# Low-power/THUNDER

Measured on AMD Instinct MI355X. Metric: particle-images/sec through expectation (box 256, 2000 rot samples), higher is better.
Workload: dtype f32 (global scan: FP32 operands split exactly into three bf16, six products -- dropped terms <= 2^-24 |w||T| each, comparable to an FP32 product's rounding -- FP32 accumulation, cancellation-guarded direct FP32 recompute; phases: FP32); 1 GPU; C3: 3D refine box 256, 2000 rotation x 151 translation global scan at rU=24 (nPxl=870) + 10 particle-filter phases (125 x 9); images_per_gpu=12500, global_batch=12500, box=256, pf=2, nR=2000, nT=151, nPxl=870, scan_algo=4, perturb_mean=acg, parallelism=dp1 (hemisphere = rank % 2)

## Files before the change

### thunder_amd/csrc/scan_split.hip

```cpp
#include "internal.h"
#include "scan_common.h"

namespace {

typedef float f32x16 __attribute__((ext_vector_type(16)));
typedef float f32x4v __attribute__((ext_vector_type(4)));
typedef __bf16 bf16x8 __attribute__((ext_vector_type(8)));
typedef __bf16 bf16x2 __attribute__((ext_vector_type(2)));
typedef uint32_t u32x4 __attribute__((ext_vector_type(4)));

enum Mode { BF16X3 = 0, BF16X6 = 2 };
typedef __bf16 H;
typedef bf16x8 HV;

template <int MODE> constexpr int nplane() { return MODE == BF16X6 ? 3 : 2; }

constexpr float SCAN_GUARD = 4.f;
constexpr int GCAP = 32;

constexpr int KC = 16;
static_assert(KC % 16 == 0, "whole float4 rows per thread in the stagers");
constexpr int IMG_TILE = 64;
constexpr int ROT_TILE = 8;
constexpr int THREADS = 64 * ROT_TILE;
constexpr int NWAVE = ROT_TILE;
constexpr int TROW = KC * 2 + 8;
constexpr int APITCH = KC + 2;

inline int pad_to(int v, int m) { return (v + m - 1) / m * m; }

struct Dims {
    int nImg, nR, nT, nPxl, nImgPad, nPxlPad, nTPad, nRB, nCk, nRBias;
};

Dims dims(int nImg, int nR, int nT, int nPxl)
{
    Dims d;
    d.nImg = nImg; d.nR = nR; d.nT = nT; d.nPxl = nPxl;
    d.nImgPad = pad_to(nImg, IMG_TILE);
    d.nPxlPad = pad_to(nPxl, KC);
    d.nTPad = pad_to(nT, 32);
    d.nRB = (nR + ROT_TILE - 1) / ROT_TILE;
    d.nCk = d.nPxlPad / KC;
    d.nRBias = pad_to(nR, 64);
    return d;
}

struct WS {
    float2* Ac;
    float* Bc;
    float* Aconst;
    float* bias;
    uint16_t* Thi;
    uint16_t* Tlo;
    uint16_t* Tl2;
    float2* Pc;
    float2* wRp;
    float* pM;
    float* pWT;
    float* pTf;
    size_t bytes;
};

WS carve(void* base, const Dims& d)
{
    thx::Carver c(base, ~size_t(0));
    WS w;
    w.Ac = c.take<float2>((size_t)d.nCk * d.nImgPad * APITCH);
    w.Bc = c.take<float>((size_t)d.nPxlPad * d.nImgPad);
    w.Aconst = c.take<float>(d.nImgPad);
    w.bias = c.take<float>((size_t)d.nImgPad * d.nRBias);
    w.Thi = c.take<uint16_t>((size_t)d.nCk * d.nTPad * TROW);
    w.Tlo = c.take<uint16_t>((size_t)d.nCk * d.nTPad * TROW);
    w.Tl2 = c.take<uint16_t>((size_t)d.nCk * d.nTPad * TROW);
    w.Pc = c.take<float2>((size_t)d.nCk * d.nRB * ROT_TILE * KC);
    w.wRp = c.take<float2>((size_t)d.nImg * d.nR);
    w.pM = c.take<float>((size_t)d.nRB * d.nImgPad);
    w.pWT = c.take<float>((size_t)d.nRB * d.nImgPad * d.nTPad);
    w.pTf = c.take<float>(d.nTPad);
    w.bytes = c.off + 256;
    return w;
}

template <typename H>
THX_DEV void split16(float x, H& hi, H& lo)
{
    hi = (H)x;
    lo = (H)(x - (float)hi);
}

THX_DEV void split3(float x, __bf16& hi, __bf16& mid, __bf16& lo)
{
    hi = (__bf16)x;
    const float r = x - (float)hi;
    mid = (__bf16)r;
    lo = (__bf16)(r - (float)mid);
}

typedef float f2v __attribute__((ext_vector_type(2)));
THX_DEV void split3x2(f2v x, uint32_t& hi, uint32_t& mid, uint32_t& lo)
{
    auto pk = [](float a, float b) { return __builtin_bit_cast(uint32_t, bf16x2{(__bf16)a, (__bf16)b}); };
    auto unpk = [](uint32_t v) { return f2v{__uint_as_float(v << 16), __uint_as_float(v & 0xffff0000u)}; };
    hi = pk(x.x, x.y);
    asm volatile("" : "+v"(hi));
    const f2v r = x - unpk(hi);
    mid = pk(r.x, r.y);
    asm volatile("" : "+v"(mid));
    const f2v r2 = r - unpk(mid);
    lo = pk(r2.x, r2.y);
}

__global__ void __launch_bounds__(256) k_prep_aconst(const float2* __restrict__ dat,
                                                     const float* __restrict__ sig, int nImg,
                                                     int nPxl, int nImgPad,
                                                     float* __restrict__ Aconst)
{
    const int l = blockIdx.x * 4 + (threadIdx.x >> 6);
    const int lane = threadIdx.x & 63;
    if (l >= nImgPad) return;
    float a = 0.f;
    if (l < nImg)
        for (int i = lane; i < nPxl; i += 64) {
            const size_t s = (size_t)l * nPxl + i;
            const float2 d = dat[s];
            a += sig[s] * (d.x * d.x + d.y * d.y);
        }
    a = wave_sum(a);
    if (lane == 0) Aconst[l] = a;
}

__global__ void __launch_bounds__(256) k_prep_img(const float2* __restrict__ dat,
                                                  const float* __restrict__ ctf,
                                                  const float* __restrict__ sig,
                                                  int nImg,
                                                  int nPxl, int nImgPad, int nPxlPad,
                                                  float2* __restrict__ Ac,
                                                  float* __restrict__ Bc)
{
    const long n = (long)nImgPad * nPxlPad;
    for (long q = blockIdx.x * (long)blockDim.x + threadIdx.x; q < n;
         q += (long)gridDim.x * blockDim.x) {
        const int i = (int)(q % nPxlPad), l = (int)(q / nPxlPad);
        float2 a = make_float2(0.f, 0.f);
        float b = 0.f;
        if (l < nImg && i < nPxl) {
            const size_t s = (size_t)l * nPxl + i;
            const float2 d = dat[s];
            const float c = ctf[s], sg = sig[s];
            const float k = -2.f * sg * c;
            a = make_float2(k * d.x, k * d.y);
            b = sg * c * c;
        }
        Ac[((size_t)(i / KC) * nImgPad + l) * APITCH + (i % KC)] = a;
        Bc[((size_t)(i / KC) * nImgPad + l) * KC + (i % KC)] = b;
    }
}

__global__ void __launch_bounds__(256) k_prep_pchunk(const float2* __restrict__ rotP, int nR,
                                                     int nPxl, int nRRows, int nPxlPad,
                                                     float2* __restrict__ Pc)
{
    const long n = (long)nRRows * nPxlPad;
    for (long q = blockIdx.x * (long)blockDim.x + threadIdx.x; q < n;
         q += (long)gridDim.x * blockDim.x) {
        const int i = (int)(q % nPxlPad), r = (int)(q / nPxlPad);
        Pc[((size_t)(i / KC) * nRRows + r) * KC + (i % KC)] =
            (r < nR && i < nPxl) ? rotP[(size_t)r * nPxl + i] : make_float2(0.f, 0.f);
    }
}

template <int MODE>
__global__ void __launch_bounds__(256) k_prep_tsplit(const float2* __restrict__ traP,
                                                     const double* __restrict__ pT, int nT,
                                                     int nPxl, int nTPad, int nPxlPad,
                                                     uint16_t* __restrict__ Thi,
                                                     uint16_t* __restrict__ Tlo,
                                                     uint16_t* __restrict__ Tl2,
                                                     float* __restrict__ pTf)
{
    const long n = (long)nTPad * nPxlPad;
    for (long q = blockIdx.x * (long)blockDim.x + threadIdx.x; q < n;
         q += (long)gridDim.x * blockDim.x) {
        const int i = (int)(q % nPxlPad), t = (int)(q / nPxlPad);
        const float2 v = (t < nT && i < nPxl) ? traP[(size_t)t * nPxl + i] : make_float2(0.f, 0.f);
        const size_t o = ((size_t)(i / KC) * nTPad + t) * TROW + (i % KC) * 2;
        H h, lo;
        if constexpr (MODE == BF16X6) {
            H m;
            split3(v.x, h, m, lo);
            Thi[o] = __builtin_bit_cast(uint16_t, h);
            Tlo[o] = __builtin_bit_cast(uint16_t, m);
            Tl2[o] = __builtin_bit_cast(uint16_t, lo);
            split3(v.y, h, m, lo);
            Thi[o + 1] = __builtin_bit_cast(uint16_t, h);
            Tlo[o + 1] = __builtin_bit_cast(uint16_t, m);
            Tl2[o + 1] = __builtin_bit_cast(uint16_t, lo);
        } else {
            split16(v.x, h, lo);
            Thi[o] = __builtin_bit_cast(uint16_t, h);
            Tlo[o] = __builtin_bit_cast(uint16_t, lo);
            split16(v.y, h, lo);
            Thi[o + 1] = __builtin_bit_cast(uint16_t, h);
            Tlo[o + 1] = __builtin_bit_cast(uint16_t, lo);
        }
        if (i == 0) pTf[t] = t < nT ? (float)pT[t] : 0.f;
    }
}

__global__ void __launch_bounds__(256) k_scan_bias(const float* __restrict__ Bc,
                                                   const float2* __restrict__ rotP, int nR,
                                                   int nPxl, int nImgPad, int nCk, int nRBias,
                                                   float* __restrict__ bias)
{
    __shared__ float sA[64][KC + 1];
    __shared__ float sB[64][KC + 1];
    const int l0 = blockIdx.x * 64, r0 = blockIdx.y * 64;
    const int tid = threadIdx.x, lane = tid & 63, w = tid >> 6;
    const int wi = w & 1, wr = w >> 1, n = lane & 31, h = lane >> 5;
    f32x16 acc;
#pragma unroll
    for (int j = 0; j < 16; j++) acc[j] = 0.f;
    for (int ck = 0; ck < nCk; ck++) {
#pragma unroll
        for (int v = 0; v < KC / 16; v++) {
            const int x = tid + v * 256;
            const float4 a = reinterpret_cast<const float4*>(Bc + ((size_t)ck * nImgPad + l0) * KC)[x];
            const int row = x / (KC / 4), c4 = (x % (KC / 4)) * 4;
            sA[row][c4] = a.x; sA[row][c4 + 1] = a.y; sA[row][c4 + 2] = a.z; sA[row][c4 + 3] = a.w;
        }
#pragma unroll
        for (int u = 0; u < KC / 4; u++) {
            const int x = tid + u * 256, rr = x / KC, kc = x % KC;
            const int r = r0 + rr, i = ck * KC + kc;
            float p2 = 0.f;
            if (r < nR && i < nPxl) {
                const float2 p = rotP[(size_t)r * nPxl + i];
                p2 = p.x * p.x + p.y * p.y;
            }
            sB[rr][kc] = p2;
        }
        __syncthreads();
#pragma unroll
        for (int k2 = 0; k2 < KC / 2; k2++)
            acc = __builtin_amdgcn_mfma_f32_32x32x2f32(sA[32 * wi + n][2 * k2 + h],
                                                       sB[32 * wr + n][2 * k2 + h], acc, 0, 0, 0);
        __syncthreads();
    }
#pragma unroll
    for (int j = 0; j < 16; j++) {
        const int row = (j & 3) + 8 * (j >> 2) + 4 * h;
        bias[(size_t)(l0 + 32 * wi + row) * nRBias + r0 + 32 * wr + n] = acc[j];
    }
}

template <bool MAX>
THX_DEV float half_reduce(float v)
{
    auto op = [](float a, float b) { return MAX ? fmaxf(a, b) : a + b; };
    v = op(v, __int_as_float(__builtin_amdgcn_update_dpp(0, __float_as_int(v), 0xb1, 0xf, 0xf, false)));
    v = op(v, __int_as_float(__builtin_amdgcn_update_dpp(0, __float_as_int(v), 0x4e, 0xf, 0xf, false)));
    v = op(v, __int_as_float(__builtin_amdgcn_update_dpp(0, __float_as_int(v), 0x124, 0xf, 0xf, false)));
    v = op(v, __int_as_float(__builtin_amdgcn_update_dpp(0, __float_as_int(v), 0x128, 0xf, 0xf, false)));
    const auto sw = __builtin_amdgcn_permlane16_swap(__float_as_uint(v), __float_as_uint(v), false, false);
    return op(__uint_as_float(sw[0]), __uint_as_float(sw[1]));
}

constexpr int SCAN_STAGES = 2;

template <int N>
THX_DEV void wait_vm()
{
    asm volatile("s_waitcnt vmcnt(%0)" ::"n"(N) : "memory");
}

template <int MODE, int NF>
struct Smem {
    static constexpr int NTP = NF * 32;
    static constexpr int NPLANE = nplane<MODE>();
    static constexpr int T_H = NTP * TROW;
    static constexpr int A_F2 = IMG_TILE * APITCH;
    static constexpr int P_F2 = ROT_TILE * KC;
    static constexpr int T_PC = T_H * 2 / 16;
    static constexpr int A_PC = A_F2 * 8 / 16;
    static constexpr int TQ = (T_PC + 63) / 64;
    static constexpr int AQ = (A_PC + 63) / 64;
    static constexpr int P_PC = P_F2 * 8 / 16;
    static constexpr int PQ = (P_PC + 63) / 64;
    static constexpr int NQ = NPLANE * TQ + AQ + PQ;
    static constexpr int TL_OFF = TQ * 1024;
    static constexpr int TL2_OFF = 2 * TQ * 1024;
    static constexpr int A_OFF = NPLANE * TQ * 1024;
    static constexpr int P_OFF = (NPLANE * TQ + AQ) * 1024;
    static constexpr int STAGE_B = NQ * 1024;
    static constexpr int EPI_B = (ROT_TILE * 64 * 3 + 64 + ROT_TILE * 8 * NTP + ROT_TILE * GCAP) * 4;
    static constexpr int TOTAL_B = SCAN_STAGES * STAGE_B > EPI_B ? SCAN_STAGES * STAGE_B : EPI_B;
};

THX_DEV void dma16(const void* g, void* ldsBase)
{
    __builtin_amdgcn_global_load_lds(
        (const __attribute__((address_space(1))) void*)g,
        (__attribute__((address_space(3))) void*)ldsBase, 16, 0, 0);
}

THX_DEV float direct_dvp(const float2* __restrict__ dat,
                                                      const float* __restrict__ ctf,
                                                      const float* __restrict__ sig,
                                                      const float2* __restrict__ traP,
                                                      const float2* __restrict__ rotP,
                                                      int nPxl, int l, int r, int t)
{
#pragma clang fp contract(off)
    const int lane = threadIdx.x & 63;
    const float2* D = dat + (size_t)l * nPxl;
    const float* C = ctf + (size_t)l * nPxl;
    const float* S = sig + (size_t)l * nPxl;
    const float2* Tt = traP + (size_t)t * nPxl;
    const float2* Pr = rotP + (size_t)r * nPxl;
    float acc = 0.f;
    for (int i = lane; i < nPxl; i += 64) {
        const float2 tp = Tt[i], p = Pr[i], d = D[i];
        const float c = C[i], sg = S[i];
        const float pr = tp.x * p.x - tp.y * p.y;
        const float pi = tp.x * p.y + tp.y * p.x;
        const float er = d.x - c * pr;
        const float ei = d.y - c * pi;
        acc += (er * er + ei * ei) * sg;
    }
    return wave_sum(acc);
}

struct Guard {
    const float2* dat;
    const float* ctf;
    const float* sig;
    const float2* traP;
    const float2* rotP;
    float kmax;
    float* dvpOut;
};

template <int NA, int NF, typename LR>
THX_DEV void guard_tile(f32x16 (&acc)[NA][NF], const Guard& gd, const float* sABr,
                        const float* sBiasr, float* sVal, LR lr, int nT, int nPxl)
{
    static_assert(NA * 16 <= 32, "one bit per (a, j) in a 32-bit word");
    const int lane = threadIdx.x & 63, n = lane & 31, h = lane >> 5;
    unsigned fw[NF];
#pragma unroll
    for (int f = 0; f < NF; f++) fw[f] = 0;
#pragma unroll
    for (int a = 0; a < NA; a++)
#pragma unroll
        for (int j = 0; j < 16; j++) {
            const int row = a * 32 + (j & 3) + 8 * (j >> 2) + 4 * h;
            const float b = sBiasr[row], ab = sABr[row];
            const bool ok = lr(row).x >= 0;
#pragma unroll
            for (int f = 0; f < NF; f++) {
                const float d = acc[a][f][j];
                const float x = d - b;
                if (ok && f * 32 + n < nT && ab + fabsf(x) > gd.kmax * fabsf(d))
                    fw[f] |= 1u << (a * 16 + j);
            }
        }
    unsigned any = 0;
#pragma unroll
    for (int f = 0; f < NF; f++) any |= fw[f];
    while (__ballot(any != 0)) {
        unsigned pw[NF];
#pragma unroll
        for (int f = 0; f < NF; f++) pw[f] = 0;
        int cnt = 0;
        for (int q = 0; q < NA * 16 && cnt < GCAP; q++) {
#pragma unroll
            for (int f = 0; f < NF; f++) {
                uint64_t m = __ballot((fw[f] >> q) & 1u);
                while (m && cnt < GCAP) {
                    const int L = __builtin_ctzll(m);
                    const int j = q & 15;
                    const int2 sm = lr((q >> 4) * 32 + (j & 3) + 8 * (j >> 2) + 4 * (L >> 5));
                    const float v = direct_dvp(gd.dat, gd.ctf, gd.sig, gd.traP, gd.rotP, nPxl, sm.x,
                                               sm.y, f * 32 + (L & 31));
                    if (lane == 0) sVal[cnt] = v;
                    if (lane == L) {
                        fw[f] &= ~(1u << q);
                        pw[f] |= 1u << q;
                    }
                    cnt++;
                    m &= m - 1;
                }
            }
        }
        __builtin_amdgcn_fence(__ATOMIC_RELEASE, "wavefront");
        __builtin_amdgcn_wave_barrier();
        int base = 0;
#pragma unroll
        for (int a = 0; a < NA; a++)
#pragma unroll
            for (int j = 0; j < 16; j++)
#pragma unroll
                for (int f = 0; f < NF; f++) {
                    const bool mine = (pw[f] >> (a * 16 + j)) & 1u;
                    const uint64_t m = __ballot(mine);
                    if (m) {
                        if (mine)
                            acc[a][f][j] = sVal[base + __builtin_amdgcn_mbcnt_hi(
                                (unsigned)(m >> 32), __builtin_amdgcn_mbcnt_lo((unsigned)m, 0))];
                        base += __builtin_popcountll(m);
                    }
                }
        __builtin_amdgcn_wave_barrier();
        any = 0;
#pragma unroll
        for (int f = 0; f < NF; f++) any |= fw[f];
    }
}

template <int MODE, int NF>
__global__ void __launch_bounds__(THREADS) __attribute__((amdgpu_waves_per_eu(2))) k_scan_split(const float2* __restrict__ Ac,
                                                        const float* __restrict__ Aconst,
                                                        const float* __restrict__ bias,
                                                        const uint16_t* __restrict__ Thi,
                                                        const uint16_t* __restrict__ Tlo,
                                                        const uint16_t* __restrict__ Tl2,
                                                        const float2* __restrict__ Pc,
                                                        const float* __restrict__ pTf,
                                                        const double* __restrict__ pR,
                                                        int nImg, int nR, int nT, int nPxl,
                                                        int nImgPad, int nPxlPad, int nTPad,
                                                        int nRBias, int nIT,
                                                        float2* __restrict__ wRp,
                                                        float* __restrict__ pM,
                                                        float* __restrict__ pWT, Guard gd)
{
    using S = Smem<MODE, NF>;
    constexpr int NTP = S::NTP;
    extern __shared__ __attribute__((aligned(16))) char lds[];

    const int tid = threadIdx.x, lane = tid & 63, w = tid >> 6;
    const int n = lane & 31, h = lane >> 5;
    const int nB = nIT * ((nR + ROT_TILE - 1) / ROT_TILE);
    const int per = (nB + 7) / 8;
    const int pq = (blockIdx.x % 8) * per + blockIdx.x / 8;
    if (pq >= nB) return;
    const int nRBk = (nR + ROT_TILE - 1) / ROT_TILE;
    const int l0 = (pq / nRBk) * IMG_TILE;
    const int rb = pq % nRBk;
    const int r = rb * ROT_TILE + w;
    const bool rValid = r < nR;

    f32x16 acc[2][NF];
#pragma unroll
    for (int a = 0; a < 2; a++)
#pragma unroll
        for (int f = 0; f < NF; f++)
#pragma unroll
            for (int j = 0; j < 16; j++) acc[a][f][j] = 0.f;

    constexpr int QS = (S::NQ + NWAVE - 1) / NWAVE;
    const int wu = __builtin_amdgcn_readfirstlane(w);
    const char* dmaG[QS];
    size_t dmaStride[QS];
    int dmaN[QS];
    {
        const size_t tStride = (size_t)nTPad * TROW * 2;
#pragma unroll
        for (int u = 0; u < QS; u++) {
            const int q = u * NWAVE + wu;
            const char* g = nullptr;
            size_t st = 0;
            int pc = 0, lim = 0;
            if (q < S::TQ) {
                g = reinterpret_cast<const char*>(Thi); st = tStride; pc = q * 64; lim = S::T_PC;
            } else if (S::NPLANE >= 2 && q < 2 * S::TQ) {
                g = reinterpret_cast<const char*>(Tlo); st = tStride; pc = (q - S::TQ) * 64; lim = S::T_PC;
            } else if (S::NPLANE >= 3 && q < 3 * S::TQ) {
                g = reinterpret_cast<const char*>(Tl2); st = tStride; pc = (q - 2 * S::TQ) * 64; lim = S::T_PC;
            } else if (q < S::NQ - S::PQ) {
                g = reinterpret_cast<const char*>(Ac + (size_t)l0 * APITCH);
                st = (size_t)nImgPad * APITCH * sizeof(float2);
                pc = (q - S::NPLANE * S::TQ) * 64; lim = S::A_PC;
            } else if (q < S::NQ) {
                g = reinterpret_cast<const char*>(Pc + (size_t)rb * ROT_TILE * KC);
                st = (size_t)nRBk * ROT_TILE * KC * sizeof(float2);
                pc = (q - (S::NQ - S::PQ)) * 64; lim = S::P_PC;
            }
            dmaG[u] = g + (size_t)pc * 16;
            dmaStride[u] = st;
            dmaN[u] = q < S::NQ ? min(64, lim - pc) : 0;
        }
    }
    const unsigned laneB = (unsigned)lane * 16u;
    auto issue_chunk = [&](int ck, char* stage) {
#pragma unroll
        for (int u = 0; u < QS; u++)
            if (lane < dmaN[u])
                dma16(dmaG[u] + (size_t)ck * dmaStride[u] + laneB, stage + (u * NWAVE + wu) * 1024);
    };
    auto stage_at = [&](int ck) { return lds + (ck % SCAN_STAGES) * S::STAGE_B; };
    const int nCk = nPxlPad / KC;
    constexpr int QLO = S::NQ / NWAVE, QREM = S::NQ % NWAVE;
    const bool qHi = w < QREM;
    auto wait_ahead = [&](int ahead) {
        if (SCAN_STAGES == 3 && ahead == 1) {
            if (qHi) wait_vm<QLO + 1>(); else wait_vm<QLO>();
        } else {
            wait_vm<0>();
        }
    };
#pragma unroll
    for (int k = 0; k < SCAN_STAGES - 1; k++)
        if (k < nCk) issue_chunk(k, stage_at(k));
    wait_ahead(nCk > 1 && SCAN_STAGES == 3 ? 1 : 0);
    __syncthreads();
    for (int ck = 0; ck < nCk; ck++) {
        const bool more = ck + SCAN_STAGES - 1 < nCk;
        if (more) issue_chunk(ck + SCAN_STAGES - 1, stage_at(ck + SCAN_STAGES - 1));
        const char* stage = stage_at(ck);
        const uint16_t* sTh = reinterpret_cast<const uint16_t*>(stage);
        const uint16_t* sTl = reinterpret_cast<const uint16_t*>(stage + S::TL_OFF);
        const float2* sA = reinterpret_cast<const float2*>(stage + S::A_OFF);
        const float2* sP = reinterpret_cast<const float2*>(stage + S::P_OFF);
#pragma unroll
        for (int s = 0; s < KC / 8; s++) {
            const int px0 = 8 * s + 4 * h;
            const f32x4v p01 = *reinterpret_cast<const f32x4v*>(sP + w * KC + px0);
            const f32x4v p23 = *reinterpret_cast<const f32x4v*>(sP + w * KC + px0 + 2);
            const float pr[4] = {p01.x, p01.z, p23.x, p23.z};
            const float pi[4] = {p01.y, p01.w, p23.y, p23.w};
            auto make_w = [&](int a, HV& wh, HV& wl) {
                const float2* rowA = sA + (a * 32 + n) * APITCH + px0;
                const f32x4v a01 = *reinterpret_cast<const f32x4v*>(rowA);
                const f32x4v a23 = *reinterpret_cast<const f32x4v*>(rowA + 2);
                const float ar[4] = {a01.x, a01.z, a23.x, a23.z};
                const float ai[4] = {a01.y, a01.w, a23.y, a23.w};
#pragma unroll
                for (int qd = 0; qd < 4; qd++) {
                    const float wr = ar[qd] * pr[qd] + ai[qd] * pi[qd];
                    const float wi = ai[qd] * pr[qd] - ar[qd] * pi[qd];
                    H x0, x1;
                    split16(wr, x0, x1); wh[2 * qd] = x0; wl[2 * qd] = x1;
                    split16(wi, x0, x1); wh[2 * qd + 1] = x0; wl[2 * qd + 1] = x1;
                }
            };
            if constexpr (MODE == BF16X6) {
                const uint16_t* sT2 = reinterpret_cast<const uint16_t*>(stage + S::TL2_OFF);
                auto make_w3 = [&](int a, HV (&wq)[3]) {
                    const float2* rowA = sA + (a * 32 + n) * APITCH + px0;
                    const f32x4v a01 = *reinterpret_cast<const f32x4v*>(rowA);
                    const f32x4v a23 = *reinterpret_cast<const f32x4v*>(rowA + 2);
                    const f2v av[4] = {f2v{a01.x, a01.y}, f2v{a01.z, a01.w}, f2v{a23.x, a23.y},
                                       f2v{a23.z, a23.w}};
                    u32x4 hq, mq, lq;
#pragma unroll
                    for (int qd = 0; qd < 4; qd++) {
                        const f2v t = av[qd] * (f2v)pr[qd];
                        const f2v w = __builtin_elementwise_fma(f2v{av[qd].y, av[qd].x},
                                                                f2v{pi[qd], -pi[qd]}, t);
                        uint32_t x0, x1, x2;
                        split3x2(w, x0, x1, x2);
                        hq[qd] = x0; mq[qd] = x1; lq[qd] = x2;
                    }
                    wq[0] = __builtin_bit_cast(HV, hq);
                    wq[1] = __builtin_bit_cast(HV, mq);
                    wq[2] = __builtin_bit_cast(HV, lq);
                };
                auto mma6 = [&](f32x16& c, const HV (&wq)[3], const HV& th, const HV& tm, const HV& tl) {
                    c = __builtin_amdgcn_mfma_f32_32x32x16_bf16(wq[2], th, c, 0, 0, 0);
                    c = __builtin_amdgcn_mfma_f32_32x32x16_bf16(wq[1], tm, c, 0, 0, 0);
                    c = __builtin_amdgcn_mfma_f32_32x32x16_bf16(wq[0], tl, c, 0, 0, 0);
                    c = __builtin_amdgcn_mfma_f32_32x32x16_bf16(wq[1], th, c, 0, 0, 0);
                    c = __builtin_amdgcn_mfma_f32_32x32x16_bf16(wq[0], tm, c, 0, 0, 0);
                    c = __builtin_amdgcn_mfma_f32_32x32x16_bf16(wq[0], th, c, 0, 0, 0);
                };
                HV wp[2][3];
                make_w3(0, wp[0]);
                make_w3(1, wp[1]);
#pragma unroll
                for (int f = 0; f < NF; f++) {
                    const int row = (f * 32 + n) * TROW + 16 * s + 8 * h;
                    const HV th = *reinterpret_cast<const HV*>(sTh + row);
                    const HV tm = *reinterpret_cast<const HV*>(sTl + row);
                    const HV tl = *reinterpret_cast<const HV*>(sT2 + row);
#pragma unroll
                    for (int a = 0; a < 2; a++) mma6(acc[a][f], wp[a], th, tm, tl);
                }
            } else if constexpr (MODE == BF16X3) {
#pragma unroll
                for (int a = 0; a < 2; a++) {
                    HV wh, wl;
                    make_w(a, wh, wl);
#pragma unroll
                    for (int f = 0; f < NF; f++) {
                        const int row = (f * 32 + n) * TROW + 16 * s + 8 * h;
                        const HV th = *reinterpret_cast<const HV*>(sTh + row);
                        const HV tl = *reinterpret_cast<const HV*>(sTl + row);
                        acc[a][f] = __builtin_amdgcn_mfma_f32_32x32x16_bf16(wh, th, acc[a][f], 0, 0, 0);
                        acc[a][f] = __builtin_amdgcn_mfma_f32_32x32x16_bf16(wh, tl, acc[a][f], 0, 0, 0);
                        acc[a][f] = __builtin_amdgcn_mfma_f32_32x32x16_bf16(wl, th, acc[a][f], 0, 0, 0);
                    }
                }
            }
        }
        wait_ahead(more && SCAN_STAGES == 3 ? 1 : 0);
        __syncthreads();
    }

    float* sBias = reinterpret_cast<float*>(lds);
    float* sMax = sBias + ROT_TILE * 64;
    float* sRowM = sMax + ROT_TILE * 64;
    float* sAB = sRowM + 64;
    float* sT = sAB + ROT_TILE * 64;
    float* sGVal = sT + ROT_TILE * 8 * NTP;
    {
        const float A = Aconst[l0 + lane], B = rValid ? bias[(size_t)(l0 + lane) * nRBias + r] : 0.f;
        sBias[w * 64 + lane] = A + B;
        sAB[w * 64 + lane] = fabsf(A) + fabsf(B);
    }
    __syncthreads();

    float pTv[NF];
#pragma unroll
    for (int f = 0; f < NF; f++) pTv[f] = pTf[f * 32 + n];
    const float pRr = rValid ? (float)pR[r] : 0.f;

#pragma unroll
    for (int a = 0; a < 2; a++)
#pragma unroll
        for (int j = 0; j < 16; j++) {
            const int row = a * 32 + (j & 3) + 8 * (j >> 2) + 4 * h;
            const float b = sBias[w * 64 + row];
#pragma unroll
            for (int f = 0; f < NF; f++) acc[a][f][j] += b;
        }
    if (gd.kmax > 0.f)
        guard_tile<2, NF>(acc, gd, sAB + w * 64, sBias + w * 64, sGVal + w * GCAP,
                          [&](int row) { return make_int2(rValid && l0 + row < nImg ? l0 + row : -1, r); },
                          nT, nPxl);
#pragma unroll
    for (int a = 0; a < 2; a++)
#pragma unroll
        for (int j = 0; j < 16; j++) {
            const int row = a * 32 + (j & 3) + 8 * (j >> 2) + 4 * h;
            const int l = l0 + row;
            if (gd.dvpOut && rValid && l < nImg) {
#pragma unroll
                for (int f = 0; f < NF; f++)
                    if (f * 32 + n < nT) gd.dvpOut[((size_t)l * nR + r) * nT + f * 32 + n] = acc[a][f][j];
            }
            float mx = -INFINITY;
#pragma unroll
            for (int f = 0; f < NF; f++)
                if (f * 32 + n < nT) mx = fmaxf(mx, acc[a][f][j]);
            mx = half_reduce<true>(mx);
            if (!rValid) mx = -INFINITY;
            float sR = 0.f;
#pragma unroll
            for (int f = 0; f < NF; f++) {
                const float e = (f * 32 + n < nT && rValid) ? __expf(acc[a][f][j] - mx) : 0.f;
                acc[a][f][j] = e;
                sR += e * pTv[f];
            }
            sR = half_reduce<false>(sR);
            if (n == 0) {
                sMax[w * 64 + row] = mx;
                if (rValid && l < nImg) wRp[(size_t)l * nR + r] = make_float2(mx, sR);
            }
        }
    __syncthreads();
    if (tid < 64) {
        float M = sMax[tid];
#pragma unroll
        for (int k = 1; k < ROT_TILE; k++) M = fmaxf(M, sMax[k * 64 + tid]);
        sRowM[tid] = M;
        pM[(size_t)rb * nImgPad + l0 + tid] = M;
    }
    __syncthreads();
#pragma unroll
    for (int a = 0; a < 2; a++)
#pragma unroll
        for (int g = 0; g < 4; g++) {
#pragma unroll
            for (int jj = 0; jj < 4; jj++) {
                const int j = 4 * g + jj, mm = jj + 4 * h;
                const int row = a * 32 + 8 * g + mm;
                const float sc = rValid ? __expf(sMax[w * 64 + row] - sRowM[row]) * pRr : 0.f;
#pragma unroll
                for (int f = 0; f < NF; f++) sT[(w * 8 + mm) * NTP + f * 32 + n] = acc[a][f][j] * sc;
            }
            __syncthreads();
            for (int x = tid; x < 8 * NTP; x += THREADS) {
                const int mm = x / NTP, t = x % NTP;
                float sum = 0.f;
#pragma unroll
                for (int k = 0; k < ROT_TILE; k++) sum += sT[(k * 8 + mm) * NTP + t];
                pWT[((size_t)rb * nImgPad + l0 + a * 32 + 8 * g + mm) * NTP + t] = sum;
            }
            __syncthreads();
        }
}

__global__ void __launch_bounds__(256) k_scan_combine_bf(const float2* __restrict__ wRp,
                                                         const float* __restrict__ pM,
                                                         const float* __restrict__ pWT,
                                                         const double* __restrict__ pR, int nR,
                                                         int nT, int nTPad, int nRB, int nImgPad,
                                                         int kIdx, int nK, float* __restrict__ wC,
                                                         float* __restrict__ wR,
                                                         float* __restrict__ wT,
                                                         float* __restrict__ baseL)
{
    extern __shared__ float sScale[];
    __shared__ float sm[4];
    __shared__ double sd[4];
    const int l = blockIdx.x;
    const int lane = threadIdx.x & 63, wv = threadIdx.x >> 6;
    float m = -INFINITY;
    for (int b = threadIdx.x; b < nRB; b += blockDim.x) m = fmaxf(m, pM[(size_t)b * nImgPad + l]);
    m = wave_max(m);
    if (lane == 0) sm[wv] = m;
    __syncthreads();
    m = fmaxf(fmaxf(sm[0], sm[1]), fmaxf(sm[2], sm[3]));
    const float base = merge_baseline(l, m, kIdx, nK, nR, nT, wC, wR, wT, baseL);
    for (int b = threadIdx.x; b < nRB; b += blockDim.x)
        sScale[b] = expf(pM[(size_t)b * nImgPad + l] - base);
    __syncthreads();
    float* wTl = wT + ((size_t)l * nK + kIdx) * nT;
    for (int t = threadIdx.x; t < nT; t += blockDim.x) {
        double a = 0.0;
        for (int b = 0; b < nRB; b++)
            a += (double)(sScale[b] * pWT[((size_t)b * nImgPad + l) * nTPad + t]);
        wTl[t] = (float)a;
    }
    float* wRl = wR + ((size_t)l * nK + kIdx) * nR;
    double c = 0.0;
    for (int r = threadIdx.x; r < nR; r += blockDim.x) {
        const float2 v = wRp[(size_t)l * nR + r];
        const float x = expf(v.x - base) * v.y;
        wRl[r] = x;
        c += (double)x * pR[r];
    }
    c = wave_sum(c);
    if (lane == 0) sd[wv] = c;
    __syncthreads();
    if (threadIdx.x == 0) wC[(size_t)l * nK + kIdx] = (float)(sd[0] + sd[1] + sd[2] + sd[3]);
}

template <int MODE, int NF>
int launch_main(const WS& ws, const Dims& d, const double* pR, const Guard& gd, hipStream_t s)
{
    const int nIT = d.nImgPad / IMG_TILE;
    dim3 grid((unsigned)(8 * thx::cdiv(nIT * d.nRB, 8)));
    constexpr int lds = Smem<MODE, NF>::TOTAL_B;
    static_assert(lds <= 160 * 1024, "scan stages exceed the LDS");
    static std::atomic<unsigned> ldsSet{0};
    const int st = thx::set_max_lds(reinterpret_cast<const void*>(k_scan_split<MODE, NF>), lds, ldsSet);
    if (st != THX_OK) return st;
    hipLaunchKernelGGL((k_scan_split<MODE, NF>), grid, dim3(THREADS), lds, s, ws.Ac, ws.Aconst,
                       ws.bias, ws.Thi, ws.Tlo, ws.Tl2, ws.Pc,
                       ws.pTf, pR, d.nImg, d.nR, d.nT, d.nPxl, d.nImgPad, d.nPxlPad, d.nTPad,
                       d.nRBias, nIT, ws.wRp, ws.pM, ws.pWT, gd);
    THX_LAUNCH_CHECK();
    return THX_OK;
}

template <int MODE>
int scan_split(const float* rotP, int nR, const float* traP, int nT, const float* dat,
               const float* ctf, const float* sigRcp, int nImg, int nPxl, const double* pR,
               const double* pT, int kIdx, int nK, float* wC, float* wR, float* wT,
               float* baseL, float guard, float* dvpOut, void* workspace, size_t wsBytes,
               hipStream_t s)
{
    const Dims d = dims(nImg, nR, nT, nPxl);
    THX_CHECK_ARG(d.nRB <= 65535 && d.nRBias / 64 <= 65535, "thx_global_scan: grid too large");
    const WS ws = carve(workspace, d);
    THX_CHECK_ARG(ws.bytes <= wsBytes, "thx_global_scan: workspace too small");
    const float2* dat2 = reinterpret_cast<const float2*>(dat);
    const float2* rot2 = reinterpret_cast<const float2*>(rotP);
    hipLaunchKernelGGL(k_prep_aconst, dim3(thx::cdiv(d.nImgPad, 4)), dim3(256), 0, s, dat2, sigRcp,
                       nImg, nPxl, d.nImgPad, ws.Aconst);
    THX_LAUNCH_CHECK();
    hipLaunchKernelGGL(k_prep_img, dim3(2048), dim3(256), 0, s, dat2, ctf, sigRcp, nImg,
                       nPxl, d.nImgPad, d.nPxlPad, ws.Ac, ws.Bc);
    THX_LAUNCH_CHECK();
    hipLaunchKernelGGL(k_prep_pchunk, dim3(2048), dim3(256), 0, s, rot2, nR, nPxl,
                       d.nRB * ROT_TILE, d.nPxlPad, ws.Pc);
    THX_LAUNCH_CHECK();
    hipLaunchKernelGGL(k_prep_tsplit<MODE>, dim3(512), dim3(256), 0, s,
                       reinterpret_cast<const float2*>(traP), pT, nT, nPxl, d.nTPad, d.nPxlPad,
                       ws.Thi, ws.Tlo, ws.Tl2, ws.pTf);
    THX_LAUNCH_CHECK();
    hipLaunchKernelGGL(k_scan_bias, dim3(d.nImgPad / 64, d.nRBias / 64), dim3(256), 0, s, ws.Bc,
                       rot2, nR, nPxl, d.nImgPad, d.nCk, d.nRBias, ws.bias);
    THX_LAUNCH_CHECK();
    const Guard gd{dat2, ctf, sigRcp, reinterpret_cast<const float2*>(traP), rot2, guard, dvpOut};
    int st;
    switch (d.nTPad / 32) {
        case 1: st = launch_main<MODE, 1>(ws, d, pR, gd, s); break;
        case 2: st = launch_main<MODE, 2>(ws, d, pR, gd, s); break;
        case 3: st = launch_main<MODE, 3>(ws, d, pR, gd, s); break;
        case 4: st = launch_main<MODE, 4>(ws, d, pR, gd, s); break;
        default: st = launch_main<MODE, 5>(ws, d, pR, gd, s); break;
    }
    if (st != THX_OK) return st;
    hipLaunchKernelGGL(k_scan_combine_bf, dim3(nImg), dim3(256), sizeof(float) * d.nRB, s,
                       ws.wRp, ws.pM, ws.pWT, pR, nR, nT, d.nTPad, d.nRB, d.nImgPad, kIdx, nK,
                       wC, wR, wT, baseL);
    THX_LAUNCH_CHECK();
    return THX_OK;
}

}

namespace thx {

size_t scan_split_workspace(int nImg, int nR, int nT, int nPxl)
{
    const Dims d = dims(nImg, nR, nT, nPxl);
    if (d.nTPad > 160) return scan_mfma_workspace(nImg, nR, nT, nPxl);
    return carve(nullptr, d).bytes;
}

float scan_guard_default() { return SCAN_GUARD; }

int scan_split_algo(int algo, const float* rotP, int nR, const float* traP, int nT,
                    const float* dat, const float* ctf, const float* sigRcp, int nImg, int nPxl,
                    const double* pR, const double* pT, int kIdx, int nK, float* wC, float* wR,
                    float* wT, float* baseL, float guard, float* dvpOut, void* workspace,
                    size_t wsBytes, hipStream_t s)
{
    if (pad_to(nT, 32) > 160) {
        THX_CHECK_ARG(dvpOut == nullptr,
                      "thx_global_scan_dvp: nT = %d > 160 runs the FP32-MFMA scan, which keeps no dvp", nT);
        return scan_mfma(rotP, nR, traP, nT, dat, ctf, sigRcp, nImg, nPxl, pR, pT, kIdx, nK,
                         wC, wR, wT, baseL, workspace, wsBytes, s);
    }
    if (algo == 2)
        return scan_split<BF16X3>(rotP, nR, traP, nT, dat, ctf, sigRcp, nImg, nPxl, pR, pT, kIdx,
                                  nK, wC, wR, wT, baseL, guard, dvpOut, workspace, wsBytes, s);
    return scan_split<BF16X6>(rotP, nR, traP, nT, dat, ctf, sigRcp, nImg, nPxl, pR, pT, kIdx, nK,
                              wC, wR, wT, baseL, guard, dvpOut, workspace, wsBytes, s);
}

}
```

Measured before the change: 90140 particle-images/s.

## Swizzle LDS tiles instead of padding, batch epilogue rows, hoist dvp stores

Replaces the padded T and A row pitches in LDS with XOR swizzles, applied both in the global prep kernels and in the fragment reads, so rows pack densely and the DMA staging uses whole wave instructions without per-lane limits. The epilogue now reduces 16 rows per round instead of 8, halving its barrier rounds, and the optional dvp output store is moved out of the max/exp loop. The aim is fewer LDS bank conflicts, less wasted LDS and fewer barriers. The cost is more address arithmetic, a larger epilogue scratch buffer, and reliance on KC being 16.

```diff
diff --git a/thunder_amd/csrc/scan_split.hip b/thunder_amd/csrc/scan_split.hip
--- a/thunder_amd/csrc/scan_split.hip
+++ b/thunder_amd/csrc/scan_split.hip
@@ -24,8 +24,12 @@
 constexpr int ROT_TILE = 8;
 constexpr int THREADS = 64 * ROT_TILE;
 constexpr int NWAVE = ROT_TILE;
-constexpr int TROW = KC * 2 + 8;
-constexpr int APITCH = KC + 2;
+constexpr int TROW = KC * 2;
+constexpr int APITCH = KC;
+
+static_assert(KC == 16, "t_swz / a_swz are worked out for 64-B T rows and 128-B a rows");
+THX_DEV int t_swz(int row) { return (row >> 2) & 3; }
+THX_DEV int a_swz(int row) { return (row >> 1) & 7; }
 
 inline int pad_to(int v, int m) { return (v + m - 1) / m * m; }
 
@@ -152,7 +156,8 @@
             a = make_float2(k * d.x, k * d.y);
             b = sg * c * c;
         }
-        Ac[((size_t)(i / KC) * nImgPad + l) * APITCH + (i % KC)] = a;
+        const int k = i % KC;
+        Ac[((size_t)(i / KC) * nImgPad + l) * APITCH + (((k >> 1) ^ a_swz(l)) << 1 | (k & 1))] = a;
         Bc[((size_t)(i / KC) * nImgPad + l) * KC + (i % KC)] = b;
     }
 }
@@ -184,7 +189,8 @@
          q += (long)gridDim.x * blockDim.x) {
         const int i = (int)(q % nPxlPad), t = (int)(q / nPxlPad);
         const float2 v = (t < nT && i < nPxl) ? traP[(size_t)t * nPxl + i] : make_float2(0.f, 0.f);
-        const size_t o = ((size_t)(i / KC) * nTPad + t) * TROW + (i % KC) * 2;
+        const int k = i % KC;
+        const size_t o = ((size_t)(i / KC) * nTPad + t) * TROW + (((k >> 2) ^ t_swz(t)) << 3 | (k & 3) << 1);
         H h, lo;
         if constexpr (MODE == BF16X6) {
             H m;
@@ -266,6 +272,8 @@
     return op(__uint_as_float(sw[0]), __uint_as_float(sw[1]));
 }
 
+constexpr int EPI_ROWS = 16;
+
 constexpr int SCAN_STAGES = 2;
 
 template <int N>
@@ -283,17 +291,18 @@
     static constexpr int P_F2 = ROT_TILE * KC;
     static constexpr int T_PC = T_H * 2 / 16;
     static constexpr int A_PC = A_F2 * 8 / 16;
-    static constexpr int TQ = (T_PC + 63) / 64;
-    static constexpr int AQ = (A_PC + 63) / 64;
     static constexpr int P_PC = P_F2 * 8 / 16;
-    static constexpr int PQ = (P_PC + 63) / 64;
+    static_assert(T_PC % 64 == 0 && A_PC % 64 == 0 && P_PC % 64 == 0, "whole wave instructions per part");
+    static constexpr int TQ = T_PC / 64;
+    static constexpr int AQ = A_PC / 64;
+    static constexpr int PQ = P_PC / 64;
     static constexpr int NQ = NPLANE * TQ + AQ + PQ;
     static constexpr int TL_OFF = TQ * 1024;
     static constexpr int TL2_OFF = 2 * TQ * 1024;
     static constexpr int A_OFF = NPLANE * TQ * 1024;
     static constexpr int P_OFF = (NPLANE * TQ + AQ) * 1024;
     static constexpr int STAGE_B = NQ * 1024;
-    static constexpr int EPI_B = (ROT_TILE * 64 * 3 + 64 + ROT_TILE * 8 * NTP + ROT_TILE * GCAP) * 4;
+    static constexpr int EPI_B = (ROT_TILE * 64 * 3 + 64 + ROT_TILE * EPI_ROWS * NTP + ROT_TILE * GCAP) * 4;
     static constexpr int TOTAL_B = SCAN_STAGES * STAGE_B > EPI_B ? SCAN_STAGES * STAGE_B : EPI_B;
 };
 
@@ -463,7 +472,6 @@
     const int wu = __builtin_amdgcn_readfirstlane(w);
     const char* dmaG[QS];
     size_t dmaStride[QS];
-    int dmaN[QS];
     {
         const size_t tStride = (size_t)nTPad * TROW * 2;
 #pragma unroll
@@ -471,38 +479,45 @@
             const int q = u * NWAVE + wu;
             const char* g = nullptr;
             size_t st = 0;
-            int pc = 0, lim = 0;
+            int pc = 0;
             if (q < S::TQ) {
-                g = reinterpret_cast<const char*>(Thi); st = tStride; pc = q * 64; lim = S::T_PC;
+                g = reinterpret_cast<const char*>(Thi); st = tStride; pc = q * 64;
             } else if (S::NPLANE >= 2 && q < 2 * S::TQ) {
-                g = reinterpret_cast<const char*>(Tlo); st = tStride; pc = (q - S::TQ) * 64; lim = S::T_PC;
+                g = reinterpret_cast<const char*>(Tlo); st = tStride; pc = (q - S::TQ) * 64;
             } else if (S::NPLANE >= 3 && q < 3 * S::TQ) {
-                g = reinterpret_cast<const char*>(Tl2); st = tStride; pc = (q - 2 * S::TQ) * 64; lim = S::T_PC;
+                g = reinterpret_cast<const char*>(Tl2); st = tStride; pc = (q - 2 * S::TQ) * 64;
             } else if (q < S::NQ - S::PQ) {
                 g = reinterpret_cast<const char*>(Ac + (size_t)l0 * APITCH);
                 st = (size_t)nImgPad * APITCH * sizeof(float2);
-                pc = (q - S::NPLANE * S::TQ) * 64; lim = S::A_PC;
+                pc = (q - S::NPLANE * S::TQ) * 64;
             } else if (q < S::NQ) {
                 g = reinterpret_cast<const char*>(Pc + (size_t)rb * ROT_TILE * KC);
                 st = (size_t)nRBk * ROT_TILE * KC * sizeof(float2);
-                pc = (q - (S::NQ - S::PQ)) * 64; lim = S::P_PC;
+                pc = (q - (S::NQ - S::PQ)) * 64;
             }
             dmaG[u] = g + (size_t)pc * 16;
             dmaStride[u] = st;
-            dmaN[u] = q < S::NQ ? min(64, lim - pc) : 0;
-        }
-    }
+        }
+    }
+    constexpr int QLO = S::NQ / NWAVE, QREM = S::NQ % NWAVE;
+    const bool qHi = wu < QREM;
     const unsigned laneB = (unsigned)lane * 16u;
     auto issue_chunk = [&](int ck, char* stage) {
 #pragma unroll
         for (int u = 0; u < QS; u++)
-            if (lane < dmaN[u])
+            if (u < QLO || qHi)
                 dma16(dmaG[u] + (size_t)ck * dmaStride[u] + laneB, stage + (u * NWAVE + wu) * 1024);
     };
     auto stage_at = [&](int ck) { return lds + (ck % SCAN_STAGES) * S::STAGE_B; };
     const int nCk = nPxlPad / KC;
-    constexpr int QLO = S::NQ / NWAVE, QREM = S::NQ % NWAVE;
-    const bool qHi = w < QREM;
+    const unsigned tLane = (unsigned)n * (TROW * 2) + ((unsigned)(h ^ t_swz(n)) << 4);
+    const unsigned aLane = (unsigned)n * (APITCH * 8) + ((unsigned)((2 * h) ^ a_swz(n)) << 4);
+    auto t_at = [&](const char* plane, int f, int s) {
+        return *reinterpret_cast<const HV*>(plane + f * 32 * TROW * 2 + (tLane ^ (unsigned)(s << 5)));
+    };
+    auto a_at = [&](const char* sA, int a, int s, int e) {
+        return *reinterpret_cast<const f32x4v*>(sA + a * 32 * APITCH * 8 + (aLane ^ (unsigned)((4 * s + e) << 4)));
+    };
     auto wait_ahead = [&](int ahead) {
         if (SCAN_STAGES == 3 && ahead == 1) {
             if (qHi) wait_vm<QLO + 1>(); else wait_vm<QLO>();
@@ -519,9 +534,9 @@
         const bool more = ck + SCAN_STAGES - 1 < nCk;
         if (more) issue_chunk(ck + SCAN_STAGES - 1, stage_at(ck + SCAN_STAGES - 1));
         const char* stage = stage_at(ck);
-        const uint16_t* sTh = reinterpret_cast<const uint16_t*>(stage);
-        const uint16_t* sTl = reinterpret_cast<const uint16_t*>(stage + S::TL_OFF);
-        const float2* sA = reinterpret_cast<const float2*>(stage + S::A_OFF);
+        const char* sTh = stage;
+        const char* sTl = stage + S::TL_OFF;
+        const char* sA = stage + S::A_OFF;
         const float2* sP = reinterpret_cast<const float2*>(stage + S::P_OFF);
 #pragma unroll
         for (int s = 0; s < KC / 8; s++) {
@@ -531,9 +546,8 @@
             const float pr[4] = {p01.x, p01.z, p23.x, p23.z};
             const float pi[4] = {p01.y, p01.w, p23.y, p23.w};
             auto make_w = [&](int a, HV& wh, HV& wl) {
-                const float2* rowA = sA + (a * 32 + n) * APITCH + px0;
-                const f32x4v a01 = *reinterpret_cast<const f32x4v*>(rowA);
-                const f32x4v a23 = *reinterpret_cast<const f32x4v*>(rowA + 2);
+                const f32x4v a01 = a_at(sA, a, s, 0);
+                const f32x4v a23 = a_at(sA, a, s, 1);
                 const float ar[4] = {a01.x, a01.z, a23.x, a23.z};
                 const float ai[4] = {a01.y, a01.w, a23.y, a23.w};
 #pragma unroll
@@ -546,11 +560,10 @@
                 }
             };
             if constexpr (MODE == BF16X6) {
-                const uint16_t* sT2 = reinterpret_cast<const uint16_t*>(stage + S::TL2_OFF);
+                const char* sT2 = stage + S::TL2_OFF;
                 auto make_w3 = [&](int a, HV (&wq)[3]) {
-                    const float2* rowA = sA + (a * 32 + n) * APITCH + px0;
-                    const f32x4v a01 = *reinterpret_cast<const f32x4v*>(rowA);
-                    const f32x4v a23 = *reinterpret_cast<const f32x4v*>(rowA + 2);
+                    const f32x4v a01 = a_at(sA, a, s, 0);
+                    const f32x4v a23 = a_at(sA, a, s, 1);
                     const f2v av[4] = {f2v{a01.x, a01.y}, f2v{a01.z, a01.w}, f2v{a23.x, a23.y},
                                        f2v{a23.z, a23.w}};
                     u32x4 hq, mq, lq;
@@ -580,10 +593,9 @@
                 make_w3(1, wp[1]);
 #pragma unroll
                 for (int f = 0; f < NF; f++) {
-                    const int row = (f * 32 + n) * TROW + 16 * s + 8 * h;
-                    const HV th = *reinterpret_cast<const HV*>(sTh + row);
-                    const HV tm = *reinterpret_cast<const HV*>(sTl + row);
-                    const HV tl = *reinterpret_cast<const HV*>(sT2 + row);
+                    const HV th = t_at(sTh, f, s);
+                    const HV tm = t_at(sTl, f, s);
+                    const HV tl = t_at(sT2, f, s);
 #pragma unroll
                     for (int a = 0; a < 2; a++) mma6(acc[a][f], wp[a], th, tm, tl);
                 }
@@ -594,9 +606,8 @@
                     make_w(a, wh, wl);
 #pragma unroll
                     for (int f = 0; f < NF; f++) {
-                        const int row = (f * 32 + n) * TROW + 16 * s + 8 * h;
-                        const HV th = *reinterpret_cast<const HV*>(sTh + row);
-                        const HV tl = *reinterpret_cast<const HV*>(sTl + row);
+                        const HV th = t_at(sTh, f, s);
+                        const HV tl = t_at(sTl, f, s);
                         acc[a][f] = __builtin_amdgcn_mfma_f32_32x32x16_bf16(wh, th, acc[a][f], 0, 0, 0);
                         acc[a][f] = __builtin_amdgcn_mfma_f32_32x32x16_bf16(wh, tl, acc[a][f], 0, 0, 0);
                         acc[a][f] = __builtin_amdgcn_mfma_f32_32x32x16_bf16(wl, th, acc[a][f], 0, 0, 0);
@@ -608,12 +619,21 @@
         __syncthreads();
     }
 
+#if THX_SCAN_NOEPI
+#if defined(__HIP_DEVICE_COMPILE__)
+#pragma unroll
+    for (int a = 0; a < 2; a++)
+#pragma unroll
+        for (int f = 0; f < NF; f++) asm volatile("" ::"v"(acc[a][f]));
+#endif
+    return;
+#endif
     float* sBias = reinterpret_cast<float*>(lds);
     float* sMax = sBias + ROT_TILE * 64;
     float* sRowM = sMax + ROT_TILE * 64;
     float* sAB = sRowM + 64;
     float* sT = sAB + ROT_TILE * 64;
-    float* sGVal = sT + ROT_TILE * 8 * NTP;
+    float* sGVal = sT + ROT_TILE * EPI_ROWS * NTP;
     {
         const float A = Aconst[l0 + lane], B = rValid ? bias[(size_t)(l0 + lane) * nRBias + r] : 0.f;
         sBias[w * 64 + lane] = A + B;
@@ -639,17 +659,25 @@
         guard_tile<2, NF>(acc, gd, sAB + w * 64, sBias + w * 64, sGVal + w * GCAP,
                           [&](int row) { return make_int2(rValid && l0 + row < nImg ? l0 + row : -1, r); },
                           nT, nPxl);
+    if (gd.dvpOut && rValid) {
+#pragma unroll
+        for (int a = 0; a < 2; a++)
+#pragma unroll
+            for (int j = 0; j < 16; j++) {
+                const int l = l0 + a * 32 + (j & 3) + 8 * (j >> 2) + 4 * h;
+                if (l < nImg) {
+#pragma unroll
+                    for (int f = 0; f < NF; f++)
+                        if (f * 32 + n < nT) gd.dvpOut[((size_t)l * nR + r) * nT + f * 32 + n] = acc[a][f][j];
+                }
+            }
+    }
 #pragma unroll
     for (int a = 0; a < 2; a++)
 #pragma unroll
         for (int j = 0; j < 16; j++) {
             const int row = a * 32 + (j & 3) + 8 * (j >> 2) + 4 * h;
             const int l = l0 + row;
-            if (gd.dvpOut && rValid && l < nImg) {
-#pragma unroll
-                for (int f = 0; f < NF; f++)
-                    if (f * 32 + n < nT) gd.dvpOut[((size_t)l * nR + r) * nT + f * 32 + n] = acc[a][f][j];
-            }
             float mx = -INFINITY;
 #pragma unroll
             for (int f = 0; f < NF; f++)
@@ -678,25 +706,26 @@
         pM[(size_t)rb * nImgPad + l0 + tid] = M;
     }
     __syncthreads();
+    static_assert(EPI_ROWS % 8 == 0 && 32 % EPI_ROWS == 0, "whole 8-row accumulator groups per round");
 #pragma unroll
     for (int a = 0; a < 2; a++)
 #pragma unroll
-        for (int g = 0; g < 4; g++) {
-#pragma unroll
-            for (int jj = 0; jj < 4; jj++) {
-                const int j = 4 * g + jj, mm = jj + 4 * h;
-                const int row = a * 32 + 8 * g + mm;
+        for (int g0 = 0; g0 < 4; g0 += EPI_ROWS / 8) {
+#pragma unroll
+            for (int j = 4 * g0; j < 4 * g0 + EPI_ROWS / 2; j++) {
+                const int mm = (j & 3) + 8 * (j >> 2) + 4 * h - 8 * g0;
+                const int row = a * 32 + 8 * g0 + mm;
                 const float sc = rValid ? __expf(sMax[w * 64 + row] - sRowM[row]) * pRr : 0.f;
 #pragma unroll
-                for (int f = 0; f < NF; f++) sT[(w * 8 + mm) * NTP + f * 32 + n] = acc[a][f][j] * sc;
+                for (int f = 0; f < NF; f++) sT[(w * EPI_ROWS + mm) * NTP + f * 32 + n] = acc[a][f][j] * sc;
             }
             __syncthreads();
-            for (int x = tid; x < 8 * NTP; x += THREADS) {
+            for (int x = tid; x < EPI_ROWS * NTP; x += THREADS) {
                 const int mm = x / NTP, t = x % NTP;
                 float sum = 0.f;
 #pragma unroll
-                for (int k = 0; k < ROT_TILE; k++) sum += sT[(k * 8 + mm) * NTP + t];
-                pWT[((size_t)rb * nImgPad + l0 + a * 32 + 8 * g + mm) * NTP + t] = sum;
+                for (int k = 0; k < ROT_TILE; k++) sum += sT[(k * EPI_ROWS + mm) * NTP + t];
+                pWT[((size_t)rb * nImgPad + l0 + a * 32 + 8 * g0 + mm) * NTP + t] = sum;
             }
             __syncthreads();
         }
```

Measured after the change: 90760 particle-images/s (median of 6 runs). No clear change (+0.7%).
